# kobejean/nerf-qa

Measured on AMD Instinct MI355X. Metric: DISTS frame-pairs/s, higher is better.
Workload: dtype f16

## Files before the change

### nerf_qa_amd/csrc/nqa_api.hip

```cpp
#include <math.h>
#include <stdarg.h>
#include <string.h>

#include <thread>
#include <vector>

#include "nqa_stages.h"

namespace nqa {

static thread_local char g_err[512] = "";

void set_error(const char *fmt, ...) {
  va_list ap;
  va_start(ap, fmt);
  vsnprintf(g_err, sizeof(g_err), fmt, ap);
  va_end(ap);
}

int check_launch(const char *what) {
  hipError_t e = hipGetLastError();
  if (e != hipSuccess) {
    set_error("%s: %s", what, hipGetErrorString(e));
    return NQA_E_LAUNCH;
// ... 142 lines not shown
      m = e > m ? e : m;
      if (k > 0) {
        const size_t p = (size_t)d.h[k] * d.w[k] * kStageC[k - 1] * prec_elem_bytes(stage_prec(prec, k));
        m = p > m ? p : m;
      }
    }
    return align_up((size_t)n * m, 256);
  }
  return align_up((size_t)n * max_act_elems(H, W) * prec_elem_bytes(prec), 256);
}

static bool bad_dims(const char *who, int n, int H, int W, int prec, int chan = 512, bool mixed_ok = false,
                     int stage = -1) {
  if (n <= 0 || H <= 0 || W <= 0) {
    set_error("%s: non-positive size n=%d H=%d W=%d", who, n, H, W);
    return true;
  }
  if (!(mixed_ok ? prec_valid_pyramid(prec) : prec_valid(prec))) {
    set_error(is_mixed(prec) ? "%s: takes no mixed mode (prec %d): pass the kernel precision of the map's own stage"
                             : "%s: unknown prec %d", who, prec);
    return true;
  }
  const long eb = (long)prec_elem_bytes(stage >= 0 ? stage_prec(prec, stage) : prec);
  if (chan > 0 && (long)H * W * chan * eb >= (1L << 31)) {
    set_error("%s: map too large for 32-bit in-image byte offsets (H*W*%d channels*%d bytes >= 2^31)", who, chan,
              (int)eb);
    return true;
  }
  return false;
}

struct StatsPlan {
  StageDesc d;
  size_t doubles;
};
static StatsPlan stats_plan(int B, const int *C, const int *HW, const int (*pooled)[2], int nstage, int prec,
                            const bool *fused = nullptr) {
  StatsPlan p;
  memset(&p, 0, sizeof(p));
  long off = 0;
  int coff = 0;
  for (int k = 0; k < nstage; ++k) {
    const bool nchw = !pooled || k == 0;
    const int kp = k >= 1 ? stage_prec(prec, k - 1) : prec;
    int nblk;
    if (nchw)
      nblk = cdiv(HW[k], stats_nchw_ppb(HW[k]));
    else if (fused && fused[k])
      nblk = k == 1 ? NQA_FUSED_PART_BLOCKS_S1 : NQA_FUSED_PART_BLOCKS;
    else if (pooled[k][0])
      nblk = pool_stats_tiles(pooled[k][0], pooled[k][1], C[k], kp, B, nullptr, nullptr);
    else
      nblk = cdiv(HW[k], stats_units_per_block(HW[k], C[k], kp, B));
    p.d.part_off[k] = off;
    p.d.nblk[k] = nblk;
    p.d.hw[k] = HW[k];
    p.d.c[k] = C[k];
    p.d.coff[k] = coff;
    off += (long)B * p.d.nblk[k] * C[k] * 5;
    coff += C[k];
  }
  p.d.nstage = nstage;
  p.d.ctot = coff;
  p.doubles = (size_t)off;
  return p;
}

}

using namespace nqa;

extern "C" {

int nqa_version(void) { return NQA_VERSION; }
const char *nqa_last_error(void) { return g_err; }

int nqa_set_conv_variant(int variant) {
  Tuning &t = tuning();
  if (variant == 1024) {
    const int c = t.mixed_launches;
    t.mixed_launches = 0;
    return c;
  }
  if (variant < 0 || variant > 1023 || (variant & 3) == 3 || (variant & 768) == 768) {
    set_error("set_conv_variant: unknown variant %d", variant);
    return NQA_E_ARG;
  }
  t.conv_variant = variant & 3;
  t.stage1_variant = (variant >> 2) & 1;
  t.window_legacy = (variant & 8) != 0;
  t.first_forms = (variant & 16) != 0;
  t.no_regw128 = (variant & 32) != 0;
  t.fuse_taps = !(variant & 64);
  t.fuse_stage1 = !(variant & 128);
  t.edge_grid = (variant >> 8) & 3;
  return NQA_OK;
}

int nqa_timing_enable(int on) {
  g_timing = on != 0;
  g_used = 0;
  return NQA_OK;
}

int nqa_timing_collect(int launches[NQA_K_COUNT], double ms[NQA_K_COUNT]) {
  for (int i = 0; i < NQA_K_COUNT; ++i) {
    launches[i] = 0;
    ms[i] = 0.0;
  }
  for (int s = 0; s < g_used; ++s) {
    float t = 0.f;
    if (hipEventSynchronize(g_ev1[s]) != hipSuccess || hipEventElapsedTime(&t, g_ev0[s], g_ev1[s]) != hipSuccess) {
      set_error("timing_collect: event %d failed", s);
      g_used = 0;
      return NQA_E_LAUNCH;
    }
    launches[g_cls[s]] += 1;
    ms[g_cls[s]] += (double)t;
  }
  g_used = 0;
  return NQA_OK;
}

size_t nqa_packed_weights_bytes(int prec) {
  if (!prec_valid_pyramid(prec)) return 0;
  size_t n = layer_offset(NQA_NUM_CONVS, prec);
  if (is_mixed(prec) || prec_elem_bytes(prec) == 2 || prec == NQA_PREC_F32S)
    n = layer0_m16_offset(prec) + kW1M16Bytes * (is_mixed(prec) || prec == NQA_PREC_F32S ? 2 : 1);
  return n;
}

int nqa_pack_vgg_weights(const float *const w_host[NQA_NUM_CONVS], const float *const b_host[NQA_NUM_CONVS], int prec,
                         void *packed_host) {
  if (!w_host || !b_host || !packed_host) {
    set_error("pack_vgg_weights: null pointer");
    return NQA_E_ARG;
  }
  if (!prec_valid_pyramid(prec)) {
    set_error("pack_vgg_weights: unknown prec %d", prec);
    return NQA_E_ARG;
  }
  char *blob = static_cast<char *>(packed_host);
  memset(blob, 0, nqa_packed_weights_bytes(prec));
  {
    float *w0 = reinterpret_cast<float *>(blob + layer_offset(0, prec));
    for (int co = 0; co < 64; ++co)
      for (int c = 0; c < 3; ++c)
        for (int t = 0; t < 9; ++t) w0[(t * 3 + c) * 64 + co] = w_host[0][(co * 3 + c) * 9 + t];
    memcpy(blob + layer_bias_offset(0, prec), b_host[0], 64 * 4);
    if (!is_mixed(prec) && prec_elem_bytes(prec) == 2) {
      uint16_t *wm = reinterpret_cast<uint16_t *>(blob + layer0_mfma_offset(prec));
      for (int ky = 0; ky < 3; ++ky)
        for (int co = 0; co < 64; ++co)
          for (int hh = 0; hh < 2; ++hh)
            for (int j = 0; j < 8; ++j) {
              const int kx = 2 * hh + j / 4, c = j % 4;
              const float v = (kx < 3 && c < 3) ? w_host[0][(co * 3 + c) * 9 + ky * 3 + kx] : 0.f;
              wm[((ky * 64 + co) * 2 + hh) * 8 + j] = prec == NQA_PREC_BF16 ? f32_to_bf16(v) : f32_to_f16(v);
            }
    }
  }
  for (int l = 1; l < NQA_NUM_CONVS; ++l) {
    const ConvSpec &cs = kConvs[l];
    const int lprec = stage_prec(prec, cs.stage), nterm = layer_terms(prec, l);
    const int cpc = prec_elem_bytes(lprec) == 4 ? 4 : 8, kc = 4 * cpc;
    const int bn = 64, ncc = cs.cin / kc;
    char *dst = blob + layer_offset(l, prec);
    {
      float one = 1.f;
      memcpy(blob + layer_bias_offset(l, prec) + (size_t)cs.cout * 4, &one, 4);
    }
    if (nterm == 2) {
      const int k = weight_scale_exp(w_host[l], (size_t)cs.cout * cs.cin * 9);
      const float wscale = ldexpf(1.f, k), winv = ldexpf(1.f, -k);
      memcpy(blob + layer_bias_offset(l, prec) + (size_t)cs.cout * 4, &winv, 4);
      for (int ct = 0; ct < cs.cout / bn; ++ct)
        for (int cc = 0; cc < ncc; ++cc)
          for (int ky = 0; ky < 3; ++ky)
// ... 969 lines not shown
```

### nerf_qa_amd/csrc/nqa_common.h

```cpp
#pragma once
#include <hip/hip_runtime.h>
#include <stdint.h>
#include <stdio.h>

#include <atomic>

#include "../../include/nqa.h"

namespace nqa {

void set_error(const char *fmt, ...);
int check_launch(const char *what);

struct TimedLaunch {
  TimedLaunch(int kclass, hipStream_t s);
  ~TimedLaunch();
  int kclass;
  hipStream_t stream;
  int slot;
};

typedef __attribute__((ext_vector_type(4))) float f32x4;
typedef __attribute__((ext_vector_type(16))) float f32x16;
typedef __attribute__((ext_vector_type(8))) __bf16 bf16x8;
// ... 116 lines not shown
struct ConvSpec {
  int cin, cout, stage;
  int last;
};
static const ConvSpec kConvs[NQA_NUM_CONVS] = {
    {3, 64, 0, 0},    {64, 64, 0, 1},   {64, 128, 1, 0},  {128, 128, 1, 1}, {128, 256, 2, 0},
    {256, 256, 2, 0}, {256, 256, 2, 1}, {256, 512, 3, 0}, {512, 512, 3, 0}, {512, 512, 3, 1},
    {512, 512, 4, 0}, {512, 512, 4, 0}, {512, 512, 4, 1}};
static inline int layer_terms(int prec, int layer) {
  return kConvs[layer].stage < NQA_MIXED_STAGES(prec) ? 2 : 1;
}
static const int kChns[NQA_NUM_TAPS] = {3, 64, 128, 256, 512, 512};
static const int kChnOff[NQA_NUM_TAPS] = {0, 3, 67, 195, 451, 963};

static constexpr size_t kZeroPage = 256;
size_t layer_offset(int layer, int prec);
size_t layer_bias_offset(int layer, int prec);
size_t layer0_mfma_offset(int prec);
size_t regw_offset(int layer, int prec);
size_t layer0_m16_offset(int prec);

static inline int cdiv(int a, int b) { return (a + b - 1) / b; }
static inline size_t align_up(size_t v, size_t a) { return (v + a - 1) / a * a; }

struct StageDesc {
  long part_off[NQA_NUM_TAPS];
  int nblk[NQA_NUM_TAPS];
  int hw[NQA_NUM_TAPS];
  int c[NQA_NUM_TAPS];
  int coff[NQA_NUM_TAPS];
  int nstage;
  int ctot;
};

struct PlaneMoments {
  int k, c;
  double mx, my, vx, vy, cov, inv;
};
__device__ inline PlaneMoments plane_moments(const double *__restrict__ part, const StageDesc &d, int b, int gc, int lane) {
  PlaneMoments m;
  int k = 0;
  while (k + 1 < d.nstage && gc >= d.coff[k + 1]) ++k;
  const int c = gc - d.coff[k];
  const double *p = part + d.part_off[k] + ((size_t)b * d.nblk[k] * d.c[k] + c) * 5;
  double s[5] = {0, 0, 0, 0, 0};
  for (int blk = lane; blk < d.nblk[k]; blk += 64) {
#pragma unroll
    for (int q = 0; q < 5; ++q) s[q] += p[(size_t)blk * d.c[k] * 5 + q];
  }
#pragma unroll
  for (int q = 0; q < 5; ++q)
    for (int off = 32; off > 0; off >>= 1) s[q] += __shfl_down(s[q], off, 64);
  m.k = k;
  m.c = c;
  m.inv = 1.0 / (double)d.hw[k];
  m.mx = s[0] * m.inv;
  m.my = s[1] * m.inv;
  m.vx = s[2] * m.inv - m.mx * m.mx;
  m.vy = s[3] * m.inv - m.my * m.my;
  m.cov = s[4] * m.inv - m.mx * m.my;
  return m;
}

size_t max_act_elems(int H, int W);

int current_device();
int num_cus(const char *who);
int raise_lds_limit(const void *kernel, std::atomic<bool> *done_dev, int bytes, const char *who);
template <auto K>
static int lds_limit(int bytes, const char *who) {
  static std::atomic<bool> done_dev[64];
  return raise_lds_limit(reinterpret_cast<const void *>(K), done_dev, bytes, who);
}

struct Tuning {
  int conv_variant = 1;
  int stage1_variant = 0;
  bool window_legacy = false;
  bool first_forms = false;
  bool no_regw128 = false;
  bool fuse_taps = true;
  bool fuse_stage1 = true;
  int edge_grid = 0;
  int mixed_launches = 0;
};
Tuning &tuning();

int conv1_1(const float *x, int n, int H, int W, const void *packed, int prec, void *out, hipStream_t st);
int conv1_fused(const float *x, const float *y, int B, int n, int H, int W, const void *packed, int prec, void *out,
                hipStream_t st);
bool stage1_is_fused(int prec, int W);
int conv3x3(const void *in, int n, int H, int W, int layer, const void *packed, int prec, void *out, hipStream_t st);
int relu_mask_split16(const float *g, const void *act, int act_split, long npix, int C, void *out, hipStream_t st);
int l2pool_backward(const float *x, const void *y_split16, const float *gy, int n, int H, int W, int C, float *gx,
                    hipStream_t st);
int conv1_1_backward(const float *gm, const float *w_oihw, int n, int H, int W, float *gimg, hipStream_t st);
int relu_mask_split16_scaled(const float *g, const void *act, int act_split, int n, long pix_per_image, int C,
                             const int *kexp, void *out, hipStream_t st);
int l2pool_backward_scaled(const float *x, const float *gy, const float *g_tap, const int *ktot, int n, int H, int W,
                           int C, float *out, hipStream_t st);
int conv1_1_backward_scaled(const float *g, const void *act0_split16, const float *w_oihw, const int *kexp,
                            const int *ktot, int n, int H, int W, float *gimg, hipStream_t st);
size_t loss_stats_backward_doubles(int B, int HW, int C);
int loss_stats_backward(const float *tx, const float *ty, int B, int HW, int C, const float *g_s1, const float *g_s2,
                        long g_stride, double *ws, float *gx, float *gy, hipStream_t st);
int grad_exponent_nblk(long per_image);
int grad_exponent(const float *g, int n, long per_image, unsigned *ws, int *kexp, int *ktot, hipStream_t st);
int window_moments_forward(const float *x, const float *y, int P, int H, int W, float *out, hipStream_t st);
int window_moments_backward(const float *x, const float *y, int P, int H, int W, const float *const g[5], float *gx,
                            float *gy, hipStream_t st);
int conv3x3_split_generic(const void *in, int n, int H, int W, int cin, int cout, const void *blob, size_t bias_off,
                          int relu, void *out, hipStream_t st);
int l2pool_to_split16(const void *in_f16, int n, int H, int W, int C, void *out_split16, hipStream_t st);
int pool_stats_to_split16(const void *feat_f16, int B, int H, int W, int C, void *pooled_split16, double *part,
                          hipStream_t st);
int l2pool(const void *in, int n, int H, int W, int C, int prec, void *out, hipStream_t st);
int stats_units_per_block(int units, int C, int prec, int B);
int stats_nchw_ppb(int HW);
int pool_stats_tiles(int Ho, int Wo, int C, int prec, int B, int *tr, int *tc);
int pool_stats(const void *feat, int B, int H, int W, int C, int prec, void *pooled, double *part, hipStream_t st);
int stats_nhwc(const void *feat, int B, int HW, int C, int prec, double *part, hipStream_t st);
int stats_nchw(const float *fx, const float *fy, int B, int C, int HW, double *part, hipStream_t st);
int finalize(const double *part, const StageDesc &d, int B, float *s1, float *s2, hipStream_t st);
int group_stats_units_per_block(int units, int C, int prec, int R);
bool group_stats_nhwc_ok(int C, int prec);
int group_stats_nhwc(const void *ref, const void *ren, int R, int K, int HW, int C, int prec, double *part, hipStream_t st);
int group_stats_nchw(const float *ref, const float *ren, int R, int K, int C, int HW, double *part, hipStream_t st);
int stats_coef(const double *part, const StageDesc &d, int B, const float *g_s1, const float *g_s2, double *coef,
               hipStream_t st);
int stats_grad(const float *const fx[NQA_NUM_TAPS], const float *const fy[NQA_NUM_TAPS], int B, const int C[NQA_NUM_TAPS],
               const int HW[NQA_NUM_TAPS], const double *coef, float *const gx[NQA_NUM_TAPS], float *const gy[NQA_NUM_TAPS],
               hipStream_t st);
int score(const float *s1, const float *s2, const float *alpha, const float *beta, int B, float *out, hipStream_t st);
int nhwc_to_nchw(const void *in, int n, int HW, int C, int prec, float *out, hipStream_t st);
#define NQA_FUSED_PART_BLOCKS 256
#define NQA_FUSED_PART_BLOCKS_S1 512
int pool_seam_finish(const float *seam, void *pooled, int nimg, int strips, int Ho, int Wo, int C, hipStream_t st);
bool conv1_pool_fusable(int B, int H, int W, int blob_prec);
int conv1_pool_stats_fused(const float *x, const float *y, int B, int H, int W, const void *packed, void *pooled, float *seam,
                           double *part, hipStream_t st);
bool conv_pool_fusable(int layer, int B, int H, int W, int blob_prec, int kprec);
size_t conv_pool_seam_bytes(int B, int H, int W, int C);
int conv_pool_stats_fused(const void *in, int B, int H, int W, int layer, const void *packed, int blob_prec, void *pooled,
                          float *seam, double *part, hipStream_t st);

}
```

### nerf_qa_amd/csrc/nqa_conv1_pool.hip

```cpp
#include <type_traits>

#include "nqa_common.h"
#include "nqa_regw.h"

namespace nqa {

struct S1Geom {
  static constexpr int TH = 4, TW = 32, HWD = TW + 2, NQI = (TH + 2) * HWD;
  static constexpr int NGI = (NQI + 15) / 16, NGRP = 2 * NGI;
  static constexpr int PITCH = 160, IMG_BYTES = NQI * PITCH, SLOT = 2 * IMG_BYTES;
  static constexpr int RAWP = 40, RAW_ROWS = TH + 5, RAW_IMG = RAW_ROWS * RAWP * 8, RAW_BYTES = 2 * RAW_IMG;
  static constexpr int RAW_PX = (TH + 4) * (TW + 4);
  static constexpr int STG_SLOTS = 12 * 64;
  static constexpr int RAW_OFF = 2 * SLOT, STG_OFF = RAW_OFF + 2 * RAW_BYTES, DUMP_OFF = STG_OFF + 3 * STG_SLOTS * 4;
  static constexpr int XB_PAD = 128;
  static constexpr int LDS = DUMP_OFF + 1024;
  static_assert(LDS <= 163840, "LDS budget");
};

template <bool RAGGED>
__global__ __launch_bounds__(512) void conv1_pool_kernel(const float *__restrict__ x, const float *__restrict__ y, int B,
                                                         const char *__restrict__ w1m, const float *__restrict__ bias1,
                                                         const char *__restrict__ wreg, const float *__restrict__ bias2,
                                                         char *__restrict__ pooled, float *__restrict__ seam,
                                                         double *__restrict__ part, int H, int W, int spairs, int rows,
                                                         int total_units, int part_nblk) {
#if defined(__HIP_DEVICE_COMPILE__)
  typedef S1Geom G;
  typedef __attribute__((ext_vector_type(4))) _Float16 h4;
  typedef __attribute__((ext_vector_type(2))) _Float16 h2;
  typedef __attribute__((ext_vector_type(2))) float f2;
  constexpr int GPP = 2, NKS = 18, NI = 2, NP = 8, COUT = 64;
  constexpr int NST = 8;
  extern __shared__ __attribute__((aligned(16))) char smem[];
  const int tid = threadIdx.x, lane = tid & 63;
  const int wave = __builtin_amdgcn_readfirstlane(tid >> 6);
  const bool tail = wave >= 4;
  const int w4 = wave & 3;
  const int l15 = lane & 15, c4 = lane >> 4;
  const int cg = w4 & 1, hs = w4 >> 1;
  const int HW = H * W;
  const int Ho = (H + 1) >> 1, Wo = (W + 1) >> 1;
  const int strips = (W + 15) >> 4;

  int u_lo, u_hi;
  unit_run(total_units, u_lo, u_hi);
  if (u_lo >= u_hi) return;
  const bool warm0 = (u_lo % rows) != 0;
  const int nsteps = (u_hi - u_lo) + (warm0 ? 1 : 0);
  struct UC {
    int n, sp, ty;
  };
  UC uc[3], ucp;
  {
    int u = u_lo - (warm0 ? 1 : 0);
    uc[0].ty = u % rows;
    u /= rows;
    uc[0].sp = u % spairs;
    uc[0].n = u / spairs;
  }
  auto next_uc = [&](const UC &a) {
    UC b = a;
    if (++b.ty == rows) {
      b.ty = 0;
      if (++b.sp == spairs) {
        b.sp = 0;
        ++b.n;
      }
    }
    return b;
  };
  uc[1] = next_uc(uc[0]);
  uc[2] = next_uc(uc[1]);
  ucp = uc[0];
  char *const xb = smem + (w4 * 64 + lane) * G::PITCH + G::XB_PAD;

  if (!tail) {
    u32x4 wf[2][NKS];
#pragma unroll
    for (int i = 0; i < 2; ++i)
#pragma unroll
      for (int ks = 0; ks < NKS; ++ks)
        wf[i][ks] = *reinterpret_cast<const u32x4 *>(wreg + ((((size_t)cg * 2 + i) * NKS + ks) * 64 + lane) * 16);
    f32x4 bia[NI];
#pragma unroll
    for (int i = 0; i < NI; ++i) bia[i] = *reinterpret_cast<const f32x4 *>(bias2 + cg * 32 + i * 16 + 4 * c4);
    __builtin_amdgcn_s_waitcnt(0x0F70);
    asm volatile("s_barrier" ::: "memory");
    asm volatile("s_barrier" ::: "memory");
    asm volatile("s_waitcnt lgkmcnt(0)\n\ts_barrier" ::: "memory");
    for (int step = 0; step < nsteps; ++step) {
      const int slot_off = (step & 1) * G::SLOT;
#pragma unroll 1
      for (int pass = 0; pass < 4; ++pass) {
        int rb = slot_off + (pass * G::HWD + hs * 16 + l15) * G::PITCH + (c4 << 4);
        asm volatile("" : "+v"(rb));
        f32x4 acc[2][GPP];
#pragma unroll
        for (int i = 0; i < 2; ++i)
#pragma unroll
          for (int g = 0; g < GPP; ++g) acc[i][g] = bia[i];
        u32x4 bf[2][GPP];
        auto load_b = [&](int ks, u32x4(&b)[GPP]) {
          const int cc = ks / 9, t = ks - cc * 9, ky = t / 3, kx = t - ky * 3;
#pragma unroll
          for (int g = 0; g < GPP; ++g)
            b[g] = *reinterpret_cast<const u32x4 *>(smem + rb + (g * G::IMG_BYTES + (ky * G::HWD + kx) * G::PITCH + cc * 64));
        };
        load_b(0, bf[0]);
// ... 29 lines not shown
        *reinterpret_cast<u32x4 *>(xb + (pass & 1) * G::SLOT) = piece[0];
        *reinterpret_cast<u32x4 *>(xb + (pass & 1) * G::SLOT + 16) = piece[1];
        asm volatile("s_waitcnt lgkmcnt(0)\n\ts_barrier" ::: "memory");
      }
    }
    return;
  }

  u32x4 w1f[4][2];
  f32x4 b1v[4];
#pragma unroll
  for (int i = 0; i < 4; ++i) {
#pragma unroll
    for (int m = 0; m < 2; ++m) w1f[i][m] = *reinterpret_cast<const u32x4 *>(w1m + ((i * 2 + m) * 64 + lane) * 16);
    b1v[i] = *reinterpret_cast<const f32x4 *>(bias1 + 16 * i + 4 * c4);
  }
  const int ttid = tid - 256;
  for (int i = ttid; i < 2 * G::RAW_BYTES / 8; i += 256) reinterpret_cast<u32x2 *>(smem + G::RAW_OFF)[i] = (u32x2){0u, 0u};

  const float isd[3] = {1.f / kStd[0], 1.f / kStd[1], 1.f / kStd[2]};
  int r_img[3], r_row[3], r_col[3];
  bool r_live[3], r_ok[3] = {false, false, false};
#pragma unroll
  for (int r = 0; r < 3; ++r) {
    const int c = r * 4 + w4, p = (c % 5) * 64 + lane;
    r_img[r] = c / 5;
    r_live[r] = c < 10 && p < G::RAW_PX;
    r_row[r] = p / (G::TW + 4);
    r_col[r] = p - r_row[r] * (G::TW + 4);
  }
  auto raw_fetch = [&](const UC &c, bool real) {
    const int n = real ? c.n : 0;
    const int x0 = c.sp * G::TW, y0 = c.ty * G::TH;
#pragma unroll
    for (int r = 0; r < 3; ++r) {
      const int gy = y0 - 2 + r_row[r], gx = x0 - 2 + r_col[r];
      r_ok[r] = real && r_live[r] && (unsigned)gy < (unsigned)H && (unsigned)gx < (unsigned)W;
      const float *img = (r_img[r] ? y : x) + (size_t)n * 3 * HW;
      const __amdgpu_buffer_rsrc_t rsrc =
          __builtin_amdgcn_make_buffer_rsrc(const_cast<float *>(img), 0, 3u * (unsigned)HW * 4u, 0x00020000);
      const unsigned off = r_ok[r] ? (unsigned)((gy * W + gx) * 4) : kOOB;
#pragma unroll
      for (int c3 = 0; c3 < 3; ++c3)
        __builtin_amdgcn_raw_ptr_buffer_load_lds(
            rsrc, (lds_void_t *)(smem + G::STG_OFF + (c3 * G::STG_SLOTS + (r * 4 + w4) * 64) * 4), 4, off, c3 * HW * 4, 0, 0);
    }
  };
  auto raw_commit = [&](int buf) {
#pragma unroll
    for (int r = 0; r < 3; ++r) {
      if (r_live[r]) {
        h4 v;
#pragma unroll
        for (int c3 = 0; c3 < 3; ++c3) {
          const float raw = *reinterpret_cast<const float *>(smem + G::STG_OFF + (c3 * G::STG_SLOTS + (r * 4 + w4) * 64 + lane) * 4);
          const float d = raw - kMean[c3], q0 = d * isd[c3], q1 = fmaf(fmaf(-q0, kStd[c3], d), isd[c3], q0);
          v[c3] = (_Float16)(r_ok[r] ? q1 : 0.f);
        }
        v[3] = (_Float16)0.f;
        *reinterpret_cast<h4 *>(smem + G::RAW_OFF + buf * G::RAW_BYTES + r_img[r] * G::RAW_IMG +
                                (r_row[r] * G::RAWP + r_col[r]) * 8) = v;
      }
    }
  };

  int c11_y0 = 0, c11_x0 = 0, c11_par = 0;
  bool c11_real = false;
  auto c11_set = [&](const UC &c, bool real, int step) {
    c11_real = real;
    c11_y0 = c.ty * G::TH;
    c11_x0 = c.sp * G::TW;
    c11_par = step & 1;
  };
  int t_raw[7], t_dst[7], t_yx[7];
#pragma unroll
  for (int j = 0; j < 7; ++j) {
    const int gi = w4 + 4 * j;
    const int img = gi >= G::NGI ? 1 : 0, q = (gi - img * G::NGI) * 16 + l15, qc = q < G::NQI ? q : G::NQI - 1;
    const int hy = qc / G::HWD, hx = qc - hy * G::HWD;
    t_yx[j] = (hy << 8) | hx;
    t_raw[j] = G::RAW_OFF + img * G::RAW_IMG + (c4 & 1) * 16 + ((hy + (c4 >> 1)) * G::RAWP + hx) * 8;
    t_dst[j] = (gi < G::NGRP && q < G::NQI) ? img * G::IMG_BYTES + q * G::PITCH + (c4 << 3) : -1;
  }
  auto c11_groups = [&](int j0, auto ng_tag) {
    constexpr int NG = decltype(ng_tag)::value;
    int dst[NG];
    unsigned mask[NG];
    u32x4 bfr[NG][2];
    f32x4 a1[NG][4];
#pragma unroll
    for (int u = 0; u < NG; ++u) {
      const int j = j0 + u;
      const int gy = c11_y0 - 1 + (t_yx[j] >> 8), gx = c11_x0 - 1 + (t_yx[j] & 255);
      const bool inside = ((unsigned)gy < (unsigned)H) & ((unsigned)gx < (unsigned)W);
      mask[u] = inside ? 0xFFFFFFFFu : 0u;
      dst[u] = (c11_real & (t_dst[j] >= 0)) ? c11_par * G::SLOT + t_dst[j] : G::DUMP_OFF + lane * 8;
      const unsigned rawb = (unsigned)(t_raw[j] + c11_par * G::RAW_BYTES);
#pragma unroll
      for (int m = 0; m < 2; ++m) {
        const char *rp = smem + rawb + m * (2 * G::RAWP * 8);
        const u32x2 lo = *reinterpret_cast<const u32x2 *>(rp), hi = *reinterpret_cast<const u32x2 *>(rp + 8);
        bfr[u][m] = (u32x4){lo[0], lo[1], hi[0], hi[1]};
      }
    }
#pragma unroll
    for (int i = 0; i < 4; ++i)
#pragma unroll
      for (int u = 0; u < NG; ++u)
        a1[u][i] = __builtin_amdgcn_mfma_f32_16x16x32_f16(__builtin_bit_cast(f16x8, w1f[i][0]), __builtin_bit_cast(f16x8, bfr[u][0]), b1v[i], 0, 0, 0);
#pragma unroll
    for (int i = 0; i < 4; ++i)
#pragma unroll
      for (int u = 0; u < NG; ++u)
        a1[u][i] = __builtin_amdgcn_mfma_f32_16x16x32_f16(__builtin_bit_cast(f16x8, w1f[i][1]), __builtin_bit_cast(f16x8, bfr[u][1]), a1[u][i], 0, 0, 0);
    const h2 z = {(_Float16)0.f, (_Float16)0.f};
#pragma unroll
    for (int u = 0; u < NG; ++u)
#pragma unroll
      for (int i = 0; i < 4; ++i) {
        const h2 lo = __builtin_elementwise_max(__builtin_convertvector((f2){a1[u][i][0], a1[u][i][1]}, h2), z);
        const h2 hi = __builtin_elementwise_max(__builtin_convertvector((f2){a1[u][i][2], a1[u][i][3]}, h2), z);
        const u32x2 vv = {__builtin_bit_cast(unsigned, lo) & mask[u], __builtin_bit_cast(unsigned, hi) & mask[u]};
        *reinterpret_cast<u32x2 *>(smem + dst[u] + (i >> 1) * 64 + (i & 1) * 32) = vv;
      }
  };
  typedef std::integral_constant<int, 2> Two;
  typedef std::integral_constant<int, 1> One;

  float U[NI][GPP][4];
  float piv[NP], s1x[NP], s1y[NP], s2x[NP], s2y[NP], sxy[NP], n_lane = 0.f;
#pragma unroll
  for (int i = 0; i < NI; ++i)
#pragma unroll
    for (int g = 0; g < GPP; ++g)
#pragma unroll
      for (int e = 0; e < 4; ++e) U[i][g][e] = 0.f;
#pragma unroll
  for (int p = 0; p < NP; ++p) piv[p] = s1x[p] = s1y[p] = s2x[p] = s2y[p] = sxy[p] = 0.f;
  const bool is15 = l15 == 15, is0 = l15 == 0, even_in = (l15 & 1) == 0 && l15 != 0;
  const size_t nimg = 2 * (size_t)B;
  const unsigned pooled_bytes = (unsigned)(nimg * Ho * Wo * COUT * 2);
  const unsigned seam_plane = (unsigned)(nimg * strips * Ho * COUT);
  const __amdgpu_buffer_rsrc_t prsrc = __builtin_amdgcn_make_buffer_rsrc(pooled, 0, pooled_bytes, 0x00020000);
  const __amdgpu_buffer_rsrc_t srsrc = __builtin_amdgcn_make_buffer_rsrc(seam, 0, 2u * seam_plane * 4u, 0x00020000);
  const unsigned y_pool_off = (unsigned)((size_t)B * Ho * Wo * COUT * 2);
  const unsigned y_seam_off = (unsigned)((size_t)B * strips * Ho * COUT);
  const int ch_lane0 = cg * 32 + 4 * c4;

  float v[NI][GPP][4];
  auto take_tile = [&](int buf) {
    typedef __attribute__((address_space(3))) const volatile u32x4 lds_cv4;
    u32x4 pc[NI];
#pragma unroll
    for (int i = 0; i < NI; ++i) pc[i] = *reinterpret_cast<lds_cv4 *>((lds_void_t *)(xb + buf * G::SLOT + i * 16));
#pragma unroll
    for (int i = 0; i < NI; ++i)
#pragma unroll
      for (int g = 0; g < GPP; ++g) {
        const h2 lo = __builtin_bit_cast(h2, (uint32_t)pc[i][2 * g]), hi = __builtin_bit_cast(h2, (uint32_t)pc[i][2 * g + 1]);
        v[i][g][0] = (float)lo[0];
        v[i][g][1] = (float)lo[1];
        v[i][g][2] = (float)hi[0];
        v[i][g][3] = (float)hi[1];
      }
  };
  auto stats_tile = [&](float vmask) {
    n_lane += RAGGED ? vmask : 1.f;
#pragma unroll
    for (int p = 0; p < NP; ++p) {
      const int i = p >> 2, e = p & 3;
      float dx = v[i][0][e] - piv[p], dy = v[i][1][e] - piv[p];
      if constexpr (RAGGED) {
        dx *= vmask;
        dy *= vmask;
      }
      s1x[p] += dx;
      s1y[p] += dy;
      s2x[p] = fmaf(dx, dx, s2x[p]);
      s2y[p] = fmaf(dy, dy, s2y[p]);
      sxy[p] = fmaf(dx, dy, sxy[p]);
    }
  };
  auto pool_even = [&](float vmask) {
#pragma unroll
    for (int i = 0; i < NI; ++i)
#pragma unroll
      for (int g = 0; g < GPP; ++g)
#pragma unroll
        for (int e = 0; e < 4; ++e) {
          const float m = RAGGED ? v[i][g][e] * vmask : v[i][g][e];
          U[i][g][e] = fmaf(2.f * m, m, U[i][g][e]);
        }
  };
  auto pool_odd = [&](float vmask, unsigned po_lane, unsigned so_lane) {
#pragma unroll
    for (int i = 0; i < NI; ++i) {
      h4 outh[GPP];
      f32x4 seamv[GPP];
#pragma unroll
      for (int g = 0; g < GPP; ++g)
#pragma unroll
        for (int e = 0; e < 4; ++e) {
          const float m = RAGGED ? v[i][g][e] * vmask : v[i][g][e];
          const float sq = m * m;
          const float u = U[i][g][e] + sq;
          const float a = u + dpp_row_shr1(u);
          const float pv = a + dpp_row_shl1(a);
          seamv[g][e] = is15 ? u : pv;
          outh[g][e] = (_Float16)__builtin_amdgcn_sqrtf(fmaf(pv, 0.0625f, 1e-12f));
          U[i][g][e] = sq;
        }
#pragma unroll
      for (int g = 0; g < GPP; ++g) {
        const unsigned po = po_lane + (g ? y_pool_off : 0u) + (unsigned)(i * 16) * 2u;
        __builtin_amdgcn_raw_buffer_store_b64(__builtin_bit_cast(u32x2, outh[g]), prsrc, po, 0, 0);
        const unsigned so = so_lane + (g ? y_seam_off * 4u : 0u) + (unsigned)(i * 16) * 4u;
        __builtin_amdgcn_raw_buffer_store_b128(__builtin_bit_cast(u32x4, seamv[g]), srsrc, so, 0, 0);
      }
    }
  };
  const unsigned lane_po = even_in ? (unsigned)(((l15 >> 1) * COUT + ch_lane0) * 2) : kOOB;
  const unsigned lane_so0 = is0 ? (unsigned)ch_lane0 * 4u : kOOB;
  const unsigned lane_so15 = is15 ? (seam_plane + (unsigned)(Ho * COUT) + (unsigned)ch_lane0) * 4u : kOOB;
  auto pool_offsets = [&](const UC &c, int j, bool emit, unsigned &po_lane, unsigned &so_lane) {
    const int s16 = c.sp * 2 + hs, x0 = s16 * 16, oy = ((c.ty * G::TH) >> 1) + j, ox0 = x0 >> 1;
    const bool live = emit && oy < Ho && x0 < W;
    const unsigned pool_row = (((unsigned)c.n * (unsigned)Ho + (unsigned)oy) * (unsigned)Wo + (unsigned)ox0) * (COUT * 2u);
    const unsigned seam_row = (((unsigned)c.n * (unsigned)strips + (unsigned)s16) * (unsigned)Ho + (unsigned)oy) * (COUT * 4u);
    const bool right = s16 + 1 < strips;
    po_lane = live ? lane_po + pool_row : kOOB;
    if constexpr (RAGGED) po_lane = (ox0 + (l15 >> 1) < Wo) ? po_lane : kOOB;
    so_lane = live ? (right ? (is15 ? lane_so15 : lane_so0) : lane_so0) + seam_row : kOOB;
  };
  auto row_mask = [&](const UC &c, int pass) -> float {
    if constexpr (!RAGGED) return 1.f;
    const int x0 = (c.sp * 2 + hs) * 16, y0 = c.ty * G::TH;
    return (y0 + pass < H && x0 + l15 < W) ? 1.f : 0.f;
  };
  auto reset_stats = [&]() {
#pragma unroll
    for (int p = 0; p < NP; ++p) {
      piv[p] = v[p >> 2][0][p & 3];
      s1x[p] = s1y[p] = s2x[p] = s2y[p] = sxy[p] = 0.f;
    }
    n_lane = 0.f;
  };
  auto flush_stats = [&](int n) {
#pragma unroll
    for (int p = 0; p < NP; ++p) {
      const int i = p >> 2, e = p & 3;
      const double pv = piv[p], nn = n_lane, ax = s1x[p], ay = s1y[p];
      double r[5] = {ax + nn * pv, ay + nn * pv, (double)s2x[p] + 2.0 * pv * ax + nn * pv * pv,
                     (double)s2y[p] + 2.0 * pv * ay + nn * pv * pv, (double)sxy[p] + pv * ax + pv * ay + nn * pv * pv};
#pragma unroll
      for (int s5 = 0; s5 < 5; ++s5) {
#pragma unroll
        for (int m = 8; m >= 1; m >>= 1) r[s5] += __shfl_xor(r[s5], m, 16);
      }
      if (l15 == 0) {
        const int c = ch_lane0 + i * 16 + e;
        double *dst = part + (((size_t)n * part_nblk + 2 * blockIdx.x + hs) * COUT + c) * 5;
#pragma unroll
        for (int s5 = 0; s5 < 5; ++s5) dst[s5] = r[s5];
      }
    }
  };

  asm volatile("s_waitcnt lgkmcnt(0)\n\ts_barrier" ::: "memory");
  raw_fetch(uc[0], true);
  asm volatile("s_waitcnt vmcnt(0)" ::: "memory");
  raw_commit(0);
  raw_fetch(uc[1], 1 < nsteps);
  asm volatile("s_waitcnt vmcnt(0)" ::: "memory");
  raw_commit(1);
  asm volatile("s_waitcnt lgkmcnt(0)\n\ts_barrier" ::: "memory");
  c11_set(uc[0], true, 0);
  c11_groups(0, Two());
  c11_groups(2, Two());
  c11_groups(4, Two());
  c11_groups(6, One());
  asm volatile("s_waitcnt lgkmcnt(0)\n\ts_barrier" ::: "memory");

  int flush_n = -1;
  bool have_prev = false;
  for (int step = 0; step < nsteps; ++step) {
    const int n = uc[0].n;
    const bool warm = warm0 && step == 0;
    const bool fresh = step == (warm0 ? 1 : 0);
    const bool change = !fresh && !warm && n != flush_n;
    bool flushed = false;
    raw_fetch(uc[2], step + 2 < nsteps);
    c11_set(uc[1], step + 1 < nsteps, step + 1);
#pragma unroll
    for (int pass = 0; pass < 4; ++pass) {
#ifdef NQA_S1_NO_EPI
      if (false) {
#else
      if (have_prev) {
#endif
        take_tile((pass + 1) & 1);
        const UC &tc = pass == 0 ? ucp : uc[0];
        const int tp = (pass + 3) & 3;
        const bool temit = pass == 0 ? !(warm0 && step == 1) : !warm;
        if (pass == 1) {
          if (uc[0].ty == 0) {
#pragma unroll
            for (int i = 0; i < NI; ++i)
#pragma unroll
              for (int g = 0; g < GPP; ++g)
#pragma unroll
                for (int e = 0; e < 4; ++e) U[i][g][e] = 0.f;
          }
          if (fresh || change) {
            if (change) {
              flush_stats(flush_n);
              flushed = true;
            }
            if (!warm) {
              reset_stats();
              flush_n = n;
            }
          }
        }
        const float vm = row_mask(tc, tp);
        stats_tile(vm);
        if (tp & 1) {
          unsigned po_lane, so_lane;
          pool_offsets(tc, tp >> 1, temit, po_lane, so_lane);
          pool_odd(vm, po_lane, so_lane);
        } else {
          pool_even(vm);
        }
      } else if (pass == 1) {
        take_tile(0);
        if (!warm) {
          reset_stats();
          flush_n = n;
        }
        stats_tile(row_mask(uc[0], 0));
        pool_even(row_mask(uc[0], 0));
      }
      if (pass >= 1) have_prev = true;
#ifndef NQA_S1_NO_C11
      if (pass == 0) c11_groups(0, Two());
      if (pass == 1) c11_groups(2, Two());
      if (pass == 2) c11_groups(4, Two());
      if (pass == 3) c11_groups(6, One());
#endif
      if (pass == 3) {
        if (flushed)
          asm volatile("s_waitcnt vmcnt(0)" ::: "memory");
        else if (step == 0)
          asm volatile("s_waitcnt vmcnt(0)" ::: "memory");
        else
          asm volatile("s_waitcnt vmcnt(%0)" ::"n"(2 * NST) : "memory");
        raw_commit(step & 1);
      }
      asm volatile("s_waitcnt lgkmcnt(0)\n\ts_barrier" ::: "memory");
    }
    ucp = uc[0];
    uc[0] = uc[1];
    uc[1] = uc[2];
    uc[2] = next_uc(uc[2]);
  }
  {
    take_tile(1);
    const float vm = row_mask(ucp, 3);
    stats_tile(vm);
    unsigned po_lane, so_lane;
    pool_offsets(ucp, 1, !(warm0 && nsteps == 1), po_lane, so_lane);
    pool_odd(vm, po_lane, so_lane);
  }
  if (flush_n >= 0) flush_stats(flush_n);
#endif
}

bool conv1_pool_fusable(int B, int H, int W, int blob_prec) {
  if (!tuning().fuse_stage1 || blob_prec != NQA_PREC_F16 || W < 16 || H < 4) return false;
  const int Ho = (H + 1) / 2, Wo = (W + 1) / 2, strips = cdiv(W, 16);
  if ((size_t)H * W * 3 * 4 >= (1ull << 31)) return false;
  if (2ull * B * Ho * Wo * 64 * 2 >= (1ull << 31)) return false;
  if (2ull * 2 * B * strips * Ho * 64 * 4 >= (1ull << 31)) return false;
  return true;
}

template <bool RAGGED>
static int launch_conv1_pool(const float *x, const float *y, int B, int H, int W, const char *packed, void *pooled, float *seam,
                             double *part, hipStream_t st) {
  typedef S1Geom G;
  if (const int rc = lds_limit<conv1_pool_kernel<RAGGED>>(G::LDS, "conv1_pool")) return rc;
  const int cus = num_cus("conv1_pool");
  if (!cus) return NQA_E_LAUNCH;
  const int spairs = cdiv(W, G::TW), rows = cdiv(H, G::TH);
  const long units = (long)B * spairs * rows;
  int grid = (int)(units < cus ? units : cus);
  if (2 * grid > NQA_FUSED_PART_BLOCKS_S1) grid = NQA_FUSED_PART_BLOCKS_S1 / 2;
  if (hipMemsetAsync(part, 0, (size_t)B * NQA_FUSED_PART_BLOCKS_S1 * 64 * 5 * sizeof(double), st) != hipSuccess) {
    set_error("conv1_pool: memset of the statistics partials failed");
    return NQA_E_LAUNCH;
  }
  const float *b1 = reinterpret_cast<const float *>(packed + layer_bias_offset(0, NQA_PREC_F16));
  const float *b2 = reinterpret_cast<const float *>(packed + layer_bias_offset(1, NQA_PREC_F16));
  {
    TimedLaunch t(NQA_K_CONV, st);
    conv1_pool_kernel<RAGGED><<<grid, 512, G::LDS, st>>>(x, y, B, packed + layer0_m16_offset(NQA_PREC_F16), b1,
                                                         packed + regw_offset(1, NQA_PREC_F16), b2, static_cast<char *>(pooled),
                                                         seam, part, H, W, spairs, rows, (int)units, NQA_FUSED_PART_BLOCKS_S1);
    const int rc = check_launch("conv1_pool");
    if (rc) return rc;
  }
  return pool_seam_finish(seam, pooled, 2 * B, cdiv(W, 16), (H + 1) / 2, (W + 1) / 2, 64, st);
}

int conv1_pool_stats_fused(const float *x, const float *y, int B, int H, int W, const void *packed, void *pooled, float *seam,
                           double *part, hipStream_t st) {
  const char *p = static_cast<const char *>(packed);
  const bool ragged = (H % 4) != 0 || (W % 32) != 0;
  return ragged ? launch_conv1_pool<true>(x, y, B, H, W, p, pooled, seam, part, st)
                : launch_conv1_pool<false>(x, y, B, H, W, p, pooled, seam, part, st);
}

}
```

### nerf_qa_amd/ops.py

```python
from __future__ import annotations

import ctypes as C
import os
from typing import List, Sequence

import numpy as np
import torch

from . import _lib
from ._lib import NUM_CONVS, PREC_DTYPE, TOTAL_CHNS, check, lib, prec_id, ptr, stream_ptr

CHNS = (3, 64, 128, 256, 512, 512)
CONV_COUT = (64, 64, 128, 128, 256, 256, 256, 512, 512, 512, 512, 512, 512)
CONV_CIN = (3, 64, 64, 128, 128, 256, 256, 256, 512, 512, 512, 512, 512)
CONV_STAGE = (0, 0, 1, 1, 2, 2, 2, 3, 3, 3, 4, 4, 4)


def _need_cuda(*ts: torch.Tensor) -> torch.device:
    dev = ts[0].device
    for t in ts:
        if not t.is_cuda:
            raise _lib.NqaError("nerf_qa_amd runs on the GPU only: got a tensor on %s "
                                "(move inputs and the module to cuda; there is no CPU fallback)" % t.device)
        if t.device != dev:
# ... 322 lines not shown
    if p not in PREC_DTYPE:
        raise ValueError(f"dists_group_stats: prec {p} is not one of the kernel-level modes")
    want = torch.float32 if nchw else PREC_DTYPE[p]
    if feat.dim() != 3 or r <= 0 or k <= 0 or feat.shape[0] != r + r * k or feat.numel() == 0 or feat.dtype != want \
            or not feat.is_contiguous():
        raise ValueError(f"dists_group_stats: expected contiguous {want} ({r + r * k}, "
                         f"{'C, HW' if nchw else 'HW, C'}), got {feat.dtype} {tuple(feat.shape)}")
    c, hw = (int(feat.shape[1]), int(feat.shape[2])) if nchw else (int(feat.shape[2]), int(feat.shape[1]))
    s1 = torch.empty((r * k, c), dtype=torch.float32, device=dev)
    s2 = torch.empty((r * k, c), dtype=torch.float32, device=dev)
    nbytes = lib().nqa_dists_group_stats_bytes(r, k, hw, c, p, int(nchw))
    scratch = torch.empty(max(nbytes, 256), dtype=torch.uint8, device=dev)
    _call(dev, lib().nqa_dists_group_stats, ptr(feat), r, k, hw, c, p, int(nchw), ptr(scratch), nbytes, ptr(s1), ptr(s2),
          stream_ptr(dev))
    return s1, s2


def _feats_args(feats0: Sequence[torch.Tensor], feats1: Sequence[torch.Tensor]):
    if len(feats0) != 6 or len(feats1) != 6:
        raise ValueError("expected six feature maps per image")
    dev = _need_cuda(*feats0, *feats1)
    f0 = [_f32c(f) for f in feats0]
    f1 = [_f32c(f) for f in feats1]
    b = f0[0].shape[0]
    for a, c in zip(f0, f1):
        if a.shape != c.shape or a.dim() != 4 or a.shape[0] != b:
            raise ValueError("feature lists disagree in shape")
    cs = (C.c_int * 6)(*[f.shape[1] for f in f0])
    hs = (C.c_int * 6)(*[f.shape[2] for f in f0])
    wsz = (C.c_int * 6)(*[f.shape[3] for f in f0])
    p0 = (C.c_void_p * 6)(*[ptr(f) for f in f0])
    p1 = (C.c_void_p * 6)(*[ptr(f) for f in f1])
    return dev, f0, f1, b, cs, hs, wsz, p0, p1


def dists_stats_nchw(feats0: Sequence[torch.Tensor], feats1: Sequence[torch.Tensor], keep_scratch: bool = False):
    dev, f0, f1, b, cs, hs, wsz, p0, p1 = _feats_args(feats0, feats1)
    ctot = sum(f.shape[1] for f in f0)
    s1 = torch.empty((b, ctot), dtype=torch.float32, device=dev)
    s2 = torch.empty((b, ctot), dtype=torch.float32, device=dev)
    nbytes = lib().nqa_stats_scratch_bytes(b, cs, hs, wsz)
    scratch = torch.empty(max(nbytes, 256), dtype=torch.uint8, device=dev)
    _call(dev, lib().nqa_dists_stats_nchw, p0, p1, b, cs, hs, wsz, ptr(scratch), scratch.numel(), ptr(s1), ptr(s2),
                                     stream_ptr(dev))
    if keep_scratch:
        return s1, s2, scratch
    return s1, s2


def dists_stats_nchw_backward(feats0: Sequence[torch.Tensor], feats1: Sequence[torch.Tensor], scratch: torch.Tensor,
                              g_s1: torch.Tensor, g_s2: torch.Tensor, need0: Sequence[bool], need1: Sequence[bool]):
    if len(need0) != 6 or len(need1) != 6:
        raise ValueError("expected six flags per list")
    dev, f0, f1, b, cs, hs, wsz, p0, p1 = _feats_args(feats0, feats1)
    _need_cuda(f0[0], scratch, g_s1, g_s2)
    ctot = sum(f.shape[1] for f in f0)
    g_s1, g_s2 = _f32c(g_s1), _f32c(g_s2)
    if tuple(g_s1.shape) != (b, ctot) or tuple(g_s2.shape) != (b, ctot):
        raise ValueError(f"expected gradients of shape {(b, ctot)}, got {tuple(g_s1.shape)} / {tuple(g_s2.shape)}")
    g0 = [torch.empty_like(f) if n else None for f, n in zip(f0, need0)]
    g1 = [torch.empty_like(f) if n else None for f, n in zip(f1, need1)]
    coef = torch.empty(max(lib().nqa_stats_backward_bytes(b, cs), 256), dtype=torch.uint8, device=dev)
    q0 = (C.c_void_p * 6)(*[None if g is None else ptr(g) for g in g0])
    q1 = (C.c_void_p * 6)(*[None if g is None else ptr(g) for g in g1])
    _call(dev, lib().nqa_dists_stats_nchw_backward, p0, p1, b, cs, hs, wsz, ptr(scratch), scratch.numel(), ptr(g_s1),
          ptr(g_s2), ptr(coef), coef.numel(), q0, q1, stream_ptr(dev))
    return g0, g1


def dists_score(s1: torch.Tensor, s2: torch.Tensor, alpha: torch.Tensor, beta: torch.Tensor) -> torch.Tensor:
    dev = _need_cuda(s1, s2, alpha, beta)
    s1, s2 = _f32c(s1), _f32c(s2)
    a, b_ = _f32c(alpha.detach().reshape(-1)), _f32c(beta.detach().reshape(-1))
    assert s1.shape == s2.shape and s1.shape[1] == TOTAL_CHNS == a.numel() == b_.numel()
    out = torch.empty((s1.shape[0],), dtype=torch.float32, device=dev)
    _call(dev, lib().nqa_dists_score, ptr(s1), ptr(s2), ptr(a), ptr(b_), s1.shape[0], ptr(out), stream_ptr(dev))
    return out


DEFAULT_CONV_VARIANT = 1


CONV_PLAIN_GRID, CONV_MIXED_GRID = 256, 512


def set_conv_variant(v: int) -> None:
    check(lib().nqa_set_conv_variant(int(v)))


def mixed_grid_launches() -> int:
    n = lib().nqa_set_conv_variant(1024)
    if n < 0:
        check(n)
    return n


def dists_fused_taps(b: int, h: int, w: int, prec) -> tuple:
    f = (C.c_int * 6)()
    check(lib().nqa_dists_fused_taps(int(b), int(h), int(w), prec_id(prec), f))
    return tuple(k for k in range(6) if f[k])


def timing_enable(on: bool) -> None:
    check(lib().nqa_timing_enable(1 if on else 0))


def timing_collect():
    n = (C.c_int * len(_lib.K_NAMES))()
    ms = (C.c_double * len(_lib.K_NAMES))()
    check(lib().nqa_timing_collect(n, ms))
    return {name: (n[i], ms[i]) for i, name in enumerate(_lib.K_NAMES)}


def adists_forward(x: torch.Tensor, y: torch.Tensor, packed: torch.Tensor, prec, ws: Workspace | None = None,
                   with_map: bool = False):
    p = prec_id(prec)
    dev = _need_cuda(x, y, packed)
    x, y = _f32c(x), _f32c(y)
    if x.shape != y.shape or x.dim() != 4 or x.shape[1] != 3:
        raise ValueError(f"expected two (B,3,H,W) tensors of equal shape, got {tuple(x.shape)} / {tuple(y.shape)}")
    b, _, h, w = x.shape
    mb = _max_pairs(lambda n: lib().nqa_adists_workspace_bytes(n, h, w, p), b)
    if mb < b:
        parts = [adists_forward(x[i:i + mb], y[i:i + mb], packed, prec, ws, with_map) for i in range(0, b, mb)]
        if with_map:
            return torch.cat([q[0] for q in parts]), torch.cat([q[1] for q in parts])
        return torch.cat(parts)
    d = torch.empty((b,), dtype=torch.float32, device=dev)
    nbytes = lib().nqa_adists_workspace_bytes(b, h, w, p)
    buf = (ws or Workspace()).get(nbytes, dev)
    if with_map:
        m = torch.empty((b, h, w), dtype=torch.float32, device=dev)
        _call(dev, lib().nqa_adists_forward_map, ptr(x), ptr(y), b, h, w, ptr(packed), p, ptr(buf), buf.numel(), ptr(d),
                                           ptr(m), stream_ptr(dev))
        return d, m
    _call(dev, lib().nqa_adists_forward, ptr(x), ptr(y), b, h, w, ptr(packed), p, ptr(buf), buf.numel(), ptr(d),
                                   stream_ptr(dev))
    return d


def adists_dists_forward(x: torch.Tensor, y: torch.Tensor, packed: torch.Tensor, prec, ws: Workspace | None = None,
                         with_map: bool = False):
    p = prec_id(prec)
    dev = _need_cuda(x, y, packed)
    x, y = _f32c(x), _f32c(y)
    if x.shape != y.shape or x.dim() != 4 or x.shape[1] != 3:
        raise ValueError(f"expected two (B,3,H,W) tensors of equal shape, got {tuple(x.shape)} / {tuple(y.shape)}")
    b, _, h, w = x.shape
    mb = _max_pairs(lambda n: lib().nqa_adists_workspace_bytes(n, h, w, p), b)
    if mb < b:
        parts = [adists_dists_forward(x[i:i + mb], y[i:i + mb], packed, prec, ws, with_map) for i in range(0, b, mb)]
        return tuple(torch.cat([q[j] for q in parts]) for j in range(4 if with_map else 3))
    d = torch.empty((b,), dtype=torch.float32, device=dev)
    s1 = torch.empty((b, TOTAL_CHNS), dtype=torch.float32, device=dev)
    s2 = torch.empty((b, TOTAL_CHNS), dtype=torch.float32, device=dev)
    m = torch.empty((b, h, w), dtype=torch.float32, device=dev) if with_map else None
    nbytes = lib().nqa_adists_workspace_bytes(b, h, w, p)
    buf = (ws or Workspace()).get(nbytes, dev)
    _call(dev, lib().nqa_adists_dists_forward, ptr(x), ptr(y), b, h, w, ptr(packed), p, ptr(buf), buf.numel(), ptr(d),
          ptr(s1), ptr(s2), ptr(m) if with_map else None, stream_ptr(dev))
    return (d, s1, s2, m) if with_map else (d, s1, s2)


def _window_stage_dims(fx: torch.Tensor, fy: torch.Tensor, q: torch.Tensor, wgt: torch.Tensor, p: int, strip: int):
    if p not in PREC_DTYPE:
        raise ValueError(f"adists_window_stage: prec {p} is not one of the kernel-level modes")
# ... 421 lines not shown
```

Baseline: 468.6.

## Carry overlapping conv1_1 halo rows between stage-1 steps instead of recomputing

In the fused conv1_1+pool stage-1 kernel, consecutive row tiles overlap by two halo rows. Instead of recomputing conv1_1 for those rows, the kernel now copies the already-computed records from the previous LDS slot into the next one and only computes the new groups. This cuts conv1_1 MFMA work per step in exchange for an extra LDS copy and more divergent per-wave group assignment. The old recompute path stays available behind a variant flag.

```diff
diff --git a/nerf_qa_amd/csrc/nqa_api.hip b/nerf_qa_amd/csrc/nqa_api.hip
--- a/nerf_qa_amd/csrc/nqa_api.hip
+++ b/nerf_qa_amd/csrc/nqa_api.hip
@@ -248,7 +248,7 @@
     t.mixed_launches = 0;
     return c;
   }
-  if (variant < 0 || variant > 1023 || (variant & 3) == 3 || (variant & 768) == 768) {
+  if (variant < 0 || (variant & ~2048) > 1023 || (variant & 3) == 3 || (variant & 768) == 768) {
     set_error("set_conv_variant: unknown variant %d", variant);
     return NQA_E_ARG;
   }
@@ -260,6 +260,7 @@
   t.fuse_taps = !(variant & 64);
   t.fuse_stage1 = !(variant & 128);
   t.edge_grid = (variant >> 8) & 3;
+  t.s1_recompute = (variant & 2048) != 0;
   return NQA_OK;
 }
 
diff --git a/nerf_qa_amd/csrc/nqa_common.h b/nerf_qa_amd/csrc/nqa_common.h
--- a/nerf_qa_amd/csrc/nqa_common.h
+++ b/nerf_qa_amd/csrc/nqa_common.h
@@ -222,6 +222,7 @@
   bool fuse_taps = true;
   bool fuse_stage1 = true;
   int edge_grid = 0;
+  bool s1_recompute = false;
   int mixed_launches = 0;
 };
 Tuning &tuning();
diff --git a/nerf_qa_amd/csrc/nqa_conv1_pool.hip b/nerf_qa_amd/csrc/nqa_conv1_pool.hip
--- a/nerf_qa_amd/csrc/nqa_conv1_pool.hip
+++ b/nerf_qa_amd/csrc/nqa_conv1_pool.hip
@@ -24,7 +24,7 @@
                                                          const char *__restrict__ wreg, const float *__restrict__ bias2,
                                                          char *__restrict__ pooled, float *__restrict__ seam,
                                                          double *__restrict__ part, int H, int W, int spairs, int rows,
-                                                         int total_units, int part_nblk) {
+                                                         int total_units, int part_nblk, int recompute) {
 #if defined(__HIP_DEVICE_COMPILE__)
   typedef S1Geom G;
   typedef __attribute__((ext_vector_type(4))) _Float16 h4;
@@ -220,20 +220,24 @@
     t_raw[j] = G::RAW_OFF + img * G::RAW_IMG + (c4 & 1) * 16 + ((hy + (c4 >> 1)) * G::RAWP + hx) * 8;
     t_dst[j] = (gi < G::NGRP && q < G::NQI) ? img * G::IMG_BYTES + q * G::PITCH + (c4 << 3) : -1;
   }
-  auto c11_groups = [&](int j0, auto ng_tag) {
+  struct GT {
+    int raw, dst, yx;
+  };
+  auto gt = [&](int j) { return GT{t_raw[j], t_dst[j], t_yx[j]}; };
+  auto c11_run = [&](auto ng_tag, const GT &ga, const GT &gb) {
     constexpr int NG = decltype(ng_tag)::value;
+    const GT gg[2] = {ga, gb};
     int dst[NG];
     unsigned mask[NG];
     u32x4 bfr[NG][2];
     f32x4 a1[NG][4];
 #pragma unroll
     for (int u = 0; u < NG; ++u) {
-      const int j = j0 + u;
-      const int gy = c11_y0 - 1 + (t_yx[j] >> 8), gx = c11_x0 - 1 + (t_yx[j] & 255);
+      const int gy = c11_y0 - 1 + (gg[u].yx >> 8), gx = c11_x0 - 1 + (gg[u].yx & 255);
       const bool inside = ((unsigned)gy < (unsigned)H) & ((unsigned)gx < (unsigned)W);
       mask[u] = inside ? 0xFFFFFFFFu : 0u;
-      dst[u] = (c11_real & (t_dst[j] >= 0)) ? c11_par * G::SLOT + t_dst[j] : G::DUMP_OFF + lane * 8;
-      const unsigned rawb = (unsigned)(t_raw[j] + c11_par * G::RAW_BYTES);
+      dst[u] = (c11_real & (gg[u].dst >= 0)) ? c11_par * G::SLOT + gg[u].dst : G::DUMP_OFF + lane * 8;
+      const unsigned rawb = (unsigned)(gg[u].raw + c11_par * G::RAW_BYTES);
 #pragma unroll
       for (int m = 0; m < 2; ++m) {
         const char *rp = smem + rawb + m * (2 * G::RAWP * 8);
@@ -264,6 +268,31 @@
   };
   typedef std::integral_constant<int, 2> Two;
   typedef std::integral_constant<int, 1> One;
+  auto c11_groups = [&](int j0, auto ng_tag) {
+    c11_run(ng_tag, gt(j0), gt(decltype(ng_tag)::value == 2 ? j0 + 1 : j0));
+  };
+
+  constexpr int CP_SHIFT = (G::NQI - 2 * G::HWD) * G::PITCH;
+  static_assert(CP_SHIFT == G::IMG_BYTES - 2 * G::HWD * G::PITCH, "image 1's records 0..67 follow image 0's 136..203");
+  static_assert(4 * 32 * G::PITCH + 2 * CP_SHIFT < 65536, "the copy's offsets are immediates");
+  const int cp_t = (3 - w4) * 64 + lane;
+  const int cp_a = (cp_t >> 3) * G::PITCH + (lane & 7) * 16;
+  const int cp_a2 = cp_a + 2 * 32 * G::PITCH + (cp_t >= 32 ? CP_SHIFT : 0);
+  auto carry_copy = [&](int src_par) {
+    typedef __attribute__((address_space(3))) volatile u32x4 lds_v4;
+    const int sb = src_par * G::SLOT + CP_SHIFT, db = (src_par ^ 1) * G::SLOT;
+    u32x4 t[5];
+#pragma unroll
+    for (int r = 0; r < 5; ++r) {
+      const int a = r == 2 ? cp_a2 : cp_a + r * 32 * G::PITCH + (r > 2 ? CP_SHIFT : 0);
+      if (r < 4 || w4 == 3) t[r] = *reinterpret_cast<lds_v4 *>((lds_void_t *)(smem + sb + a));
+    }
+#pragma unroll
+    for (int r = 0; r < 5; ++r) {
+      const int a = r == 2 ? cp_a2 : cp_a + r * 32 * G::PITCH + (r > 2 ? CP_SHIFT : 0);
+      if (r < 4 || w4 == 3) *reinterpret_cast<lds_v4 *>((lds_void_t *)(smem + db + a)) = t[r];
+    }
+  };
 
   float U[NI][GPP][4];
   float piv[NP], s1x[NP], s1y[NP], s2x[NP], s2y[NP], sxy[NP], n_lane = 0.f;
@@ -429,6 +458,7 @@
     bool flushed = false;
     raw_fetch(uc[2], step + 2 < nsteps);
     c11_set(uc[1], step + 1 < nsteps, step + 1);
+    const bool carry = !recompute && uc[1].ty != 0 && step + 1 < nsteps;
 #pragma unroll
     for (int pass = 0; pass < 4; ++pass) {
 #ifdef NQA_S1_NO_EPI
@@ -480,10 +510,25 @@
       }
       if (pass >= 1) have_prev = true;
 #ifndef NQA_S1_NO_C11
-      if (pass == 0) c11_groups(0, Two());
-      if (pass == 1) c11_groups(2, Two());
-      if (pass == 2) c11_groups(4, Two());
-      if (pass == 3) c11_groups(6, One());
+      if (carry) {
+        if (pass == 0) c11_run(One(), gt(1), gt(1));
+        if (pass == 1) c11_run(Two(), gt(2), gt(5));
+        if (pass == 2) {
+          if (w4 == 0)
+            c11_run(One(), gt(3), gt(3));
+          else
+            c11_run(One(), gt(4), gt(4));
+        }
+        if (pass == 3) {
+          if (w4 < 2) c11_run(One(), gt(6), gt(6));
+          carry_copy(step & 1);
+        }
+      } else {
+        if (pass == 0) c11_groups(0, Two());
+        if (pass == 1) c11_groups(2, Two());
+        if (pass == 2) c11_groups(4, Two());
+        if (pass == 3) c11_groups(6, One());
+      }
 #endif
       if (pass == 3) {
         if (flushed)
@@ -543,7 +588,8 @@
     TimedLaunch t(NQA_K_CONV, st);
     conv1_pool_kernel<RAGGED><<<grid, 512, G::LDS, st>>>(x, y, B, packed + layer0_m16_offset(NQA_PREC_F16), b1,
                                                          packed + regw_offset(1, NQA_PREC_F16), b2, static_cast<char *>(pooled),
-                                                         seam, part, H, W, spairs, rows, (int)units, NQA_FUSED_PART_BLOCKS_S1);
+                                                         seam, part, H, W, spairs, rows, (int)units, NQA_FUSED_PART_BLOCKS_S1,
+                                                         tuning().s1_recompute ? 1 : 0);
     const int rc = check_launch("conv1_pool");
     if (rc) return rc;
   }
diff --git a/nerf_qa_amd/ops.py b/nerf_qa_amd/ops.py
--- a/nerf_qa_amd/ops.py
+++ b/nerf_qa_amd/ops.py
@@ -428,6 +428,7 @@
 
 
 CONV_PLAIN_GRID, CONV_MIXED_GRID = 256, 512
+CONV_S1_RECOMPUTE = 2048
 
 
 def set_conv_variant(v: int) -> None:
```

New measurement: 468.3, median of 2. No clear change (-0.1%).
